# swyoon/Diffusion-by-MaxEntIRL

Measured on AMD Instinct MI355X. Metric: images/sec (CIFAR-10 DDPM T=10 generation), higher is better.
Workload: dtype bf16; 1 GPU; CIFAR-10 DDPM U-Net (35.7M params) VARSampler T=10 generation, 256 images/GPU/step, 3x32x32 (BASELINE configs[1]); noise drawn inside the step; global_batch=256, T=10, parallelism=dp1 (independent trajectories, no collective)

## Files before the change

diffusion-by-maxentirl_amd/csrc/conv_ws.hip:

```cpp
#include "conv_common.h"
#include <stdlib.h>
#include <type_traits>


#ifdef DXMI_CONV_STAMPS
__device__ unsigned g_ws_wait[256][176];
extern "C" int dxmi_debug_read_ws_stamps(void* dst, int bytes) {
    return (int)hipMemcpyFromSymbol(dst, HIP_SYMBOL(g_ws_wait), bytes, 0, hipMemcpyDeviceToHost);
}
#define WS_STAMPED_BARRIER(idx)                                                                     \
    do {                                                                                            \
        const unsigned long long t0_ = __builtin_amdgcn_s_memtime();                                \
        ws_barrier();                                                                               \
        const unsigned long long t1_ = __builtin_amdgcn_s_memtime();                                \
        if (wave == 0 && lane == 0 && (idx) < 160 && blockIdx.x < 256) g_ws_wait[blockIdx.x][(idx)] = (unsigned)(t1_ - t0_); \
    } while (0)
#define WS_CLOCKSTAMP(slot, cond)                                                                    \
    do {                                                                                            \
        if ((cond) && lane == 0 && blockIdx.x < 256) {                                              \
            g_ws_wait[blockIdx.x][(slot)] = (unsigned)__builtin_amdgcn_s_memtime();                 \
            g_ws_wait[blockIdx.x][(slot) + 1] = (unsigned)__builtin_amdgcn_s_memrealtime();         \
        }                                                                                           \
    } while (0)
#define WS_TSTAMP(slot, cond)                                                                        \
    do {                                                                                            \
        if ((cond) && lane == 0 && blockIdx.x < 256) g_ws_wait[blockIdx.x][(slot)] = (unsigned)__builtin_amdgcn_s_memtime(); \
    } while (0)
#define WS_DBG(bit) (p.stagger & (bit))
#else
#define WS_STAMPED_BARRIER(idx) ws_barrier()
#define WS_TSTAMP(slot, cond) do {} while (0)
#define WS_CLOCKSTAMP(slot, cond) do {} while (0)
#define WS_DBG(bit) 0
#endif

__device__ unsigned long long g_ws_clock[4];
extern "C" int dxmi_conv_ws_last_clock(unsigned long long* host_out4) {
    return hipMemcpyFromSymbol(host_out4, HIP_SYMBOL(g_ws_clock), 4 * sizeof(unsigned long long), 0, hipMemcpyDeviceToHost) == hipSuccess ? DXMI_OK
                                                                                                                                          : DXMI_ELAUNCH;
}

namespace {

constexpr int WS_A_SLOT = 8192;
constexpr int WS_RING = 6;
constexpr int WS_A_RING = WS_RING * WS_A_SLOT;
constexpr int WS_RO = 256 * 256;
constexpr int WS_TB = 1024;
constexpr int WS_HALO_BLOCKS = 22;
constexpr int WS_HALO = WS_HALO_BLOCKS * 1024;

__device__ uint4 ws_zero16 = {0u, 0u, 0u, 0u};

#define WS_GPTR(p) ((const __attribute__((address_space(1))) void*)(p))
#define WS_LPTR(p) ((__attribute__((address_space(3))) void*)(p))

__device__ __forceinline__ void ws_barrier() { asm volatile("s_waitcnt lgkmcnt(0)\n\ts_barrier" ::: "memory"); }

#define WS_INTERLEAVE_4()                                       \
    do {                                                        \
        _Pragma("unroll") for (int i_ = 0; i_ < 4; ++i_) {      \
            __builtin_amdgcn_sched_group_barrier(0x008, 3, 0);  \
            __builtin_amdgcn_sched_group_barrier(0x100, 1, 0);  \
        }                                                       \
        __builtin_amdgcn_sched_group_barrier(0x008, 4, 0);      \
    } while (0)
#define WS_INTERLEAVE_8()                                       \
    do {                                                        \
        _Pragma("unroll") for (int i_ = 0; i_ < 8; ++i_) {      \
            __builtin_amdgcn_sched_group_barrier(0x008, 1, 0);  \
            __builtin_amdgcn_sched_group_barrier(0x100, 1, 0);  \
        }                                                       \
        __builtin_amdgcn_sched_group_barrier(0x008, 8, 0);      \
    } while (0)

__device__ __forceinline__ void ws_wait_vm(int n) {
    switch (n >> 1) {
    case 0: asm volatile("s_waitcnt vmcnt(0)" ::: "memory"); break;
    case 1: asm volatile("s_waitcnt vmcnt(2)" ::: "memory"); break;
    case 2: asm volatile("s_waitcnt vmcnt(4)" ::: "memory"); break;
    case 3: asm volatile("s_waitcnt vmcnt(6)" ::: "memory"); break;
    case 4: asm volatile("s_waitcnt vmcnt(8)" ::: "memory"); break;
    case 5: asm volatile("s_waitcnt vmcnt(10)" ::: "memory"); break;
    case 6: asm volatile("s_waitcnt vmcnt(12)" ::: "memory"); break;
    case 7: asm volatile("s_waitcnt vmcnt(14)" ::: "memory"); break;
    case 8: asm volatile("s_waitcnt vmcnt(16)" ::: "memory"); break;
    case 9: asm volatile("s_waitcnt vmcnt(18)" ::: "memory"); break;
    case 10: asm volatile("s_waitcnt vmcnt(20)" ::: "memory"); break;
    default: asm volatile("s_waitcnt vmcnt(22)" ::: "memory"); break;
    }
}

struct WsTile {
    int cot, n0, oy0, ox0;
};

#ifdef WS_VALU_PIECES
typedef float ws_f32x2 __attribute__((ext_vector_type(2)));
struct WsValuLoad {
    u32x4 r[2];
    ws_f32x2 A[4], B[4];
    unsigned sink;
    __device__ __forceinline__ void init(int lane) {
        for (int k = 0; k < 2; ++k) r[k] = u32x4{0x3f803f00u + lane + k, 0xbf803e80u + k, 0x3e003f80u + lane, 0x40003f00u - k};
        for (int i = 0; i < 4; ++i) {
            A[i] = ws_f32x2{0.9f + 0.01f * lane, 1.1f - 0.01f * i};
            B[i] = ws_f32x2{0.05f * i, -0.03f * lane};
        }
        sink = 0;
    }
    __device__ __forceinline__ void run() {
#pragma unroll
        for (int k = 0; k < WS_VALU_PIECES; ++k) {
            u32x4& raw = r[k & 1];
#pragma unroll
            for (int i = 0; i < 4; ++i) {
                ws_f32x2 x = {__builtin_bit_cast(float, raw[i] << 16), __builtin_bit_cast(float, raw[i] & 0xffff0000u)};
                ws_f32x2 y = x * A[i] + B[i];
                const ws_f32x2 t = y * ws_f32x2{-1.4426950408889634f, -1.4426950408889634f};
                ws_f32x2 e = {__builtin_amdgcn_exp2f(t[0]), __builtin_amdgcn_exp2f(t[1])};
                e = e + ws_f32x2{1.f, 1.f};
                const ws_f32x2 rc = {__builtin_amdgcn_rcpf(e[0]), __builtin_amdgcn_rcpf(e[1])};
                y = y * rc;
                bf16x2 o = {(bf16)y[0], (bf16)y[1]};
                sink ^= __builtin_bit_cast(unsigned, o);
            }
            raw += u32x4{0x10001u, 0x20003u, 0x10002u, 0x30001u};
        }
    }
};
#define WS_VALU_DECL(lane_) WsValuLoad vl_; vl_.init(lane_)
#define WS_VALU_RUN() vl_.run()
#define WS_VALU_DONE() do { if (vl_.sink == 0x12345u) reinterpret_cast<volatile unsigned*>(p.out)[0] = vl_.sink; } while (0)
#else
#define WS_VALU_DECL(lane_) do {} while (0)
#define WS_VALU_RUN() do {} while (0)
#define WS_VALU_DONE() do {} while (0)
#endif

template <int TW>
__device__ __forceinline__ void conv_ws_body(const ConvArgs& p) {
    constexpr int TH = 256 / TW, HP = TW == 32 ? 34 : 18, HH = TH + 2, TWl = TW == 32 ? 5 : 4;
    extern __shared__ __attribute__((aligned(1024))) char smem[];
    char* const halo0 = smem;
    char* const aring = smem + 2 * WS_HALO;
    char* const ro = aring + WS_A_RING;
    float* const tb = reinterpret_cast<float*>(ro + WS_RO);

    const int tid = threadIdx.x, lane = tid & 63;
    const int wave = __builtin_amdgcn_readfirstlane(tid >> 6);
    const int txn = p.OW / TW, tyn = p.OH / TH;
    const int nchunks = (p.C0 + p.C1) / 32;
    const int S = 9 * nchunks;
    const int ntiles = p.PT * p.CT;
    const int ups = p.ups ? 1 : 0;

    auto tile_of = [&](int q, WsTile& t) {
        t.cot = q % p.CT;
        const int pt = q / p.CT;
        const int tx = pt % txn, ty = (pt / txn) % tyn;
        t.n0 = pt / (txn * tyn);
        t.oy0 = ty * TH;
        t.ox0 = tx * TW;
    };

    const int q0 = dxmi_xcd_logical(blockIdx.x, gridDim.x, p.xcd_order);
    int q = q0;
    if (q >= ntiles) return;
    const int qstride = gridDim.x;
    if (blockIdx.x == 0 && tid == 0) {
        g_ws_clock[0] = __builtin_amdgcn_s_memtime();
        g_ws_clock[1] = __builtin_amdgcn_s_memrealtime();
    }
    WS_CLOCKSTAMP(172, wave == 0);

    if (wave < 4) {
        const int ch = wave & 1, ph = wave >> 1;
        const int px = lane & 15, kg = lane >> 4;
        constexpr int BROW = TW == 32 ? 2 : 1;
        int bbase[3];
#pragma unroll
        for (int kx = 0; kx < 3; ++kx)
            bbase[kx] = ((ph * (8 / BROW) * HP + px + kx) * 64) + ((kg ^ (2 * (((px + kx) >> 2) & 1))) << 4);
        const char* const abase = aring + ch * 2048 + ((kg >> 1) * 4096) + ((px + 32 * (kg & 1)) << 4);
        f32x4 acc[4][8];
#pragma unroll
        for (int cb = 0; cb < 4; ++cb)
#pragma unroll
            for (int nb = 0; nb < 8; ++nb)
#pragma unroll
                for (int r = 0; r < 4; ++r) acc[cb][nb][r] = 0.f;
        bf16x8 A0[4], A1[4], Bx[4], By[4];
        auto read_a = [&](int u, bf16x8 (&A)[4]) {
            const char* as = abase + (u % WS_RING) * WS_A_SLOT;
#pragma unroll
            for (int cb = 0; cb < 4; ++cb) A[cb] = *reinterpret_cast<const bf16x8*>(as + (cb >> 1) * 1024 + (cb & 1) * 256);
        };
        auto read_b = [&](int u, int half, bf16x8 (&B)[4]) {
            const int t = u % 9, ky = t / 3, kx = t % 3;
            const char* hb = halo0 + ((u / 9) & 1) * WS_HALO + bbase[kx];
#pragma unroll
            for (int i = 0; i < 4; ++i) {
                const int nb = half * 4 + i;
                B[i] = *reinterpret_cast<const bf16x8*>(hb + ((nb / BROW + ky) * HP + (nb % BROW) * 16) * 64);
            }
        };
        auto mfma16 = [&](const bf16x8 (&A)[4], const bf16x8 (&B)[4], int half) {
#pragma unroll
            for (int i = 0; i < 4; ++i)
#pragma unroll
                for (int cb = 0; cb < 4; ++cb)
                    acc[cb][half * 4 + i] = __builtin_amdgcn_mfma_f32_16x16x32_bf16(A[cb], B[i], acc[cb][half * 4 + i], 0, 0, 0);
        };
        const float slope = dxmi_act_slope(p.act);
        const bool has_res = p.residual != nullptr;

        ws_barrier();
        WS_CLOCKSTAMP(168, wave == 0);
        read_a(0, A0);
        read_b(0, 0, Bx);
        int stamp_i = 0;
        (void)stamp_i;
        for (;;) {
            const bool more = q + qstride < ntiles;
            for (int c = 0; c < nchunks; c += 2) {
#pragma unroll
                for (int u = 0; u < 18; ++u) {
                    read_b(u, 1, By);
                    if (u & 1) mfma16(A1, Bx, 0); else mfma16(A0, Bx, 0);
                    WS_INTERLEAVE_4();
                    if (u % 3 == 2) { if (!(WS_DBG(16))) WS_STAMPED_BARRIER(stamp_i + c * 9 + u); }
                    if (u & 1) read_a(u + 1, A0); else read_a(u + 1, A1);
                    read_b(u + 1, 0, Bx);
                    if (u & 1) mfma16(A1, By, 1); else mfma16(A0, By, 1);
                    WS_INTERLEAVE_8();
                    __builtin_amdgcn_sched_barrier(0);
                }
            }
            WS_TSTAMP(158, wave == 0 && q == q0);
            ws_barrier();
            WS_TSTAMP(159, wave == 0 && q == q0);
            {
                const bool plain = p.act == DXMI_ACT_NONE;
                char* const rowb = ro + ((ph * 128 + px) << 8) + 8 * (kg & 1);
                const bool want_stats = p.gn_stats != nullptr;
                const int cot_ = q % p.CT;
                float* const stp = want_stats ? p.gn_stats + ((size_t)((q / p.CT) * 2 + ph) * (p.Cout >> 1) + cot_ * 64 + ch * 32 + kg * 2) * 2 : nullptr;
                auto epi = [&](auto RES, auto MASK, auto ACT, auto STATS) {
                    constexpr bool kRes = decltype(RES)::value, kMask = decltype(MASK)::value, kAct = decltype(ACT)::value, kStats = decltype(STATS)::value;
#pragma unroll
                    for (int cb = 0; cb < 4; ++cb) {
                        float st[4] = {0.f, 0.f, 0.f, 0.f};
                        const int co = ch * 64 + cb * 16 + 4 * kg;
                        const f32x4 b0 = *reinterpret_cast<const f32x4*>(tb + co), t0 = *reinterpret_cast<const f32x4*>(tb + 128 + co);
                        f32x4 bv;
#pragma unroll
                        for (int e = 0; e < 4; ++e) bv[e] = b0[e] + t0[e];
                        char* const a0 = rowb + (((ch * 8 + cb * 2 + (kg >> 1)) ^ px) << 4);
                        bf16x4 r[8];
                        if constexpr (kRes) {
#pragma unroll
                            for (int nb = 0; nb < 8; ++nb) r[nb] = *reinterpret_cast<const bf16x4*>(a0 + nb * 4096);
                        }
#pragma unroll
                        for (int nb = 0; nb < 8; ++nb) {
                            f32x4 v;
#pragma unroll
                            for (int e = 0; e < 4; ++e) v[e] = acc[cb][nb][e] + bv[e];
                            if constexpr (kRes) {
                                if constexpr (kMask) {
#pragma unroll
                                    for (int e = 0; e < 4; ++e) v[e] *= ((float)r[nb][e] > 0.f ? 1.f : p.mask_slope);
                                } else {
#pragma unroll
                                    for (int e = 0; e < 4; ++e) v[e] += (float)r[nb][e];
                                }
                            }
                            if constexpr (kAct) {
#pragma unroll
                                for (int e = 0; e < 4; ++e) v[e] = dxmi_act_lin(v[e], slope);
                            }
                            bf16x4 o;
#pragma unroll
                            for (int e = 0; e < 4; ++e) o[e] = (bf16)v[e];
                            *reinterpret_cast<bf16x4*>(a0 + nb * 4096) = o;
                            if constexpr (kStats) dxmi_stats4(o, st);
#pragma unroll
                            for (int e = 0; e < 4; ++e) acc[cb][nb][e] = 0.f;
                        }
                        if constexpr (kStats) {
#pragma unroll
                            for (int e = 0; e < 4; ++e) st[e] = dxmi_row16_sum(st[e]);
                            if (px == 0 && cot_ * 128 + co < p.Cout) {
                                f32x4 sv;
#pragma unroll
                                for (int e = 0; e < 4; ++e) sv[e] = st[e];
                                *reinterpret_cast<f32x4*>(stp + cb * 16) = sv;
                            }
                        }
                    }
                };
                using T_ = std::true_type;
                using F_ = std::false_type;
                const bool is_mask = has_res && p.res_is_mask;
                if (plain && !is_mask) {
                    if (has_res) { if (want_stats) epi(T_{}, F_{}, F_{}, T_{}); else epi(T_{}, F_{}, F_{}, F_{}); }
                    else { if (want_stats) epi(F_{}, F_{}, F_{}, T_{}); else epi(F_{}, F_{}, F_{}, F_{}); }
                } else if (!want_stats) {
                    if (is_mask) { if (plain) epi(T_{}, T_{}, F_{}, F_{}); else epi(T_{}, T_{}, T_{}, F_{}); }
                    else if (has_res) epi(T_{}, F_{}, T_{}, F_{});
                    else epi(F_{}, F_{}, T_{}, F_{});
                } else {
                    if (is_mask) epi(T_{}, T_{}, T_{}, T_{});
                    else if (has_res) epi(T_{}, F_{}, T_{}, T_{});
                    else epi(F_{}, F_{}, T_{}, T_{});
                }
            }
            WS_TSTAMP(166, wave == 0 && q == q0);
            ws_barrier();
            WS_TSTAMP(157, wave == 0 && q == q0);
// ... 50 lines not shown
        if (WS_DBG(1)) {}
        const int t2l = lw * 64 + lane, prl = t2l >> 4;
        const int lpar_l0 = prl * p.Cout + (((t2l & 15) ^ prl) * 8), lpar_l1 = prl * p.Cout + (((t2l & 15) ^ (prl | 8)) * 8);
        const int c8e_l = (t2l & 15) ^ prl, c8o_l = (t2l & 15) ^ (prl | 8);
        const int kpc_l = (32 + nchunks - 2) / (nchunks - 1);
        const char* const zero_page_l = reinterpret_cast<const char*>(p.mask_src);
        bool first_tile_l = true, first_group0 = true;
        load_group(0, cur.cot, cur.cot, fq[0]);
        load_group(1, cur.cot, cur.cot, fq[1]);
        asm volatile("s_waitcnt vmcnt(12)" ::: "memory");
        store_group(0, fq[0]);
        asm volatile("s_waitcnt lgkmcnt(0)" ::: "memory");
        load_group(2, cur.cot, cur.cot, fq[0]);
        ws_barrier();
        bool first_tile = true;
        for (;;) {
            const bool more = q + qstride < ntiles;
            WsTile nxt = cur;
            if (more) tile_of(q + qstride, nxt);
            if (!first_tile && lw == 0 && !(WS_DBG(8))) {
                const int co_a = cur.cot * 128 + lane, co_b = co_a + 64 < p.Cout ? co_a + 64 : p.Cout - 1;
                if (p.bias) {
                    __builtin_amdgcn_global_load_lds(WS_GPTR(p.bias + co_a), WS_LPTR(tb), 4, 0, 0);
                    __builtin_amdgcn_global_load_lds(WS_GPTR(p.bias + co_b), WS_LPTR(tb + 64), 4, 0, 0);
                }
                if (p.addvec) {
                    const float* av = p.addvec + (size_t)cur.n0 * p.addvec_ld;
                    __builtin_amdgcn_global_load_lds(WS_GPTR(av + co_a), WS_LPTR(tb + 128), 4, 0, 0);
                    __builtin_amdgcn_global_load_lds(WS_GPTR(av + co_b), WS_LPTR(tb + 192), 4, 0, 0);
                }
            }
            const bf16* const res_t = p.residual + ((((size_t)cur.n0 * p.OH + cur.oy0) * p.OW + cur.ox0) * p.Cout + cur.cot * 128);
            const bool res_here = !first_tile_l && p.residual != nullptr && !(WS_DBG(8));
            first_tile_l = false;
            first_tile = false;
            for (int G0 = 0; G0 < NG; G0 += 2) {
#pragma unroll
                for (int j = 0; j < 2; ++j) {
                    const int G = G0 + j;
                    if (G > 0 || first_group0) {
                        asm volatile("s_waitcnt vmcnt(12)" ::: "memory");
                        store_group(G + 1, fq[(j + 1) & 1]);
                        asm volatile("s_waitcnt lgkmcnt(0)" ::: "memory");
                    }
                    if (res_here && G > 0) {
                        const int cg = (G - 1) / 3, g3 = (G - 1) - cg * 3;
                        if (cg + 1 < nchunks) {
                            const int k0 = cg * kpc_l < 32 ? cg * kpc_l : 32, k1 = k0 + kpc_l < 32 ? k0 + kpc_l : 32;
                            const int i0 = g3 < 2 ? 3 * g3 : 6, i1 = g3 < 2 ? 3 * g3 + 3 : 12;
                            const int ka = k0 + i0 < k1 ? k0 + i0 : k1, kb = k0 + i1 < k1 ? k0 + i1 : k1;
#pragma unroll 1
                            for (int k = ka; k < kb; ++k) {
                                const int rel = ((k >> (TWl - 3)) * p.OW + (k & (TW / 8 - 1)) * 8) * p.Cout + ((k & 1) ? lpar_l1 : lpar_l0);
                                const bool ok = cur.cot * 128 + ((k & 1) ? c8o_l : c8e_l) * 8 < p.Cout;
                                const void* g = ok ? (const void*)(res_t + rel) : (const void*)zero_page_l;
                                __builtin_amdgcn_global_load_lds(WS_GPTR(g), WS_LPTR(ro + (k * 128 + lw * 64) * 16), 16, 0, 0);
                            }
                        }
                    }
                    if (G > 0 || first_group0) load_group(G + 3, cur.cot, more ? nxt.cot : cur.cot, fq[(j + 1) & 1]);
                    WS_TSTAMP(151, wave == 4 && G == 0 && q == q0 + qstride);
                    WS_VALU_RUN();
                    if (!(WS_DBG(16))) ws_barrier();
                }
            }
            first_group0 = false;
            if (more) {
                asm volatile("s_waitcnt vmcnt(12)" ::: "memory");
                store_group(1, fq[1]);
                asm volatile("s_waitcnt lgkmcnt(0)" ::: "memory");
                load_group(3, nxt.cot, nxt.cot, fq[1]);
            }
            ws_barrier();
            ws_barrier();
            WS_TSTAMP(150, wave == 4 && q == q0);
            if (!more) break;
            q += qstride;
            cur = nxt;
        }
        asm volatile("s_waitcnt vmcnt(0)" ::: "memory");
        WS_VALU_DONE();
    } else if (wave == 6) {
        WS_VALU_DECL(lane);
        constexpr int HBA = WS_HALO_BLOCKS;
        const char* const zero_page = reinterpret_cast<const char*>(p.mask_src);
        int hrel0[HBA], hrel1[HBA];
        unsigned m_in = 0, m_top = 0, m_bot = 0, m_left = 0, m_right = 0;
#pragma unroll
        for (int k = 0; k < HBA; ++k) {
            const int hp = k * 16 + (lane >> 2);
            const int hy = hp / HP, hx = hp - hy * HP;
            const int rel = ((hy - 1) >> ups) * p.IW + ((hx - 1) >> ups);
            const int j8 = ((lane & 3) ^ (2 * ((hx >> 2) & 1))) * 8;
            hrel0[k] = (rel * p.C0 + j8) * 2;
            hrel1[k] = (rel * p.C1 + j8) * 2;
            m_in |= (unsigned)(hy < HH && hx < TW + 2) << k;
            m_top |= (unsigned)(hy == 0) << k;
            m_bot |= (unsigned)(hy == HH - 1) << k;
            m_left |= (unsigned)(hx == 0) << k;
            m_right |= (unsigned)(hx == TW + 1) << k;
        }
        unsigned hmask = 0;
        int hbase0 = 0, hbase1 = 0;
        auto halo_plan = [&](const WsTile& t) {
            hmask = m_in;
            if (t.oy0 == 0) hmask &= ~m_top;
            if (t.oy0 + TH == p.OH) hmask &= ~m_bot;
            if (t.ox0 == 0) hmask &= ~m_left;
            if (t.ox0 + TW == p.OW) hmask &= ~m_right;
            const int pix = (t.n0 * p.IH + (t.oy0 >> ups)) * p.IW + (t.ox0 >> ups);
            hbase0 = pix * p.C0 * 2;
            hbase1 = pix * p.C1 * 2;
        };
        auto halo_issue = [&](int c, char* buf, int ka, int kb) {
            if (WS_DBG(2)) return;
            const int cbase = c * 32;
            const bool first = cbase < p.C0;
            const char* base = reinterpret_cast<const char*>(first ? p.in0 : p.in1) + (first ? cbase : cbase - p.C0) * 2 + (first ? hbase0 : hbase1);
#pragma unroll
            for (int k = 0; k < HBA; ++k) {
                if (k < ka || k >= kb) continue;
                const char* g = (hmask >> k) & 1 ? base + (first ? hrel0[k] : hrel1[k]) : zero_page;
                __builtin_amdgcn_global_load_lds(WS_GPTR(g), WS_LPTR(buf + k * 1024), 16, 0, 0);
            }
        };
        WsTile cur;
        tile_of(q, cur);
        if (!p.bias) { tb[lane] = 0.f; tb[64 + lane] = 0.f; }
        if (!p.addvec) { tb[128 + lane] = 0.f; tb[192 + lane] = 0.f; }
        halo_plan(cur);
        halo_issue(0, halo0, 0, HBA);
        if (!(WS_DBG(8))) {
            const int co_a = cur.cot * 128 + lane, co_b = co_a + 64 < p.Cout ? co_a + 64 : p.Cout - 1;
            if (p.bias) {
                __builtin_amdgcn_global_load_lds(WS_GPTR(p.bias + co_a), WS_LPTR(tb), 4, 0, 0);
                __builtin_amdgcn_global_load_lds(WS_GPTR(p.bias + co_b), WS_LPTR(tb + 64), 4, 0, 0);
            }
            if (p.addvec) {
                const float* av = p.addvec + (size_t)cur.n0 * p.addvec_ld;
                __builtin_amdgcn_global_load_lds(WS_GPTR(av + co_a), WS_LPTR(tb + 128), 4, 0, 0);
                __builtin_amdgcn_global_load_lds(WS_GPTR(av + co_b), WS_LPTR(tb + 192), 4, 0, 0);
            }
        }
        asm volatile("s_waitcnt vmcnt(0)" ::: "memory");
        ws_barrier();
        WsTile nxt = cur;
        for (;;) {
            const bool more = q + qstride < ntiles;
            for (int c = 0; c < nchunks; ++c) {
                const bool wrap = c + 1 == nchunks;
                if (wrap && more) {
                    tile_of(q + qstride, nxt);
                    halo_plan(nxt);
                }
                const bool do_halo = !wrap || more;
                char* const hbuf = halo0 + ((c + 1) & 1) * WS_HALO;
                const int hc = wrap ? 0 : c + 1;
#pragma unroll
                for (int t = 0; t < 9; ++t) {
                    if (t < 8 && do_halo) halo_issue(hc, hbuf, 3 * t, 3 * t + 3 < HBA ? 3 * t + 3 : HBA);
                    if (t == 8) asm volatile("s_waitcnt vmcnt(0)" ::: "memory");
                    if (t % 3 == 2) { WS_VALU_RUN(); if (!(WS_DBG(16))) ws_barrier(); }
                }
            }
            ws_barrier();
            ws_barrier();
            if (!more) break;
            q += qstride;
            cur = nxt;
        }
        WS_VALU_DONE();
    } else if (wave == 7) {
        WS_VALU_DECL(lane);
        const char* const zero_page = reinterpret_cast<const char*>(p.mask_src);
        const int prA = lane >> 4, prB = 4 + (lane >> 4), lc = lane & 15;
        const int lparA[2] = {prA * p.Cout + ((lc ^ prA) * 8), prA * p.Cout + ((lc ^ (prA | 8)) * 8)};
        const int lparB[2] = {prB * p.Cout + ((lc ^ prB) * 8), prB * p.Cout + ((lc ^ (prB | 8)) * 8)};
        const int c8A[2] = {lc ^ prA, lc ^ (prA | 8)}, c8B[2] = {lc ^ prB, lc ^ (prB | 8)};
        auto tile_base = [&](const WsTile& t) -> size_t {
            return (((size_t)t.n0 * p.OH + t.oy0) * p.OW + t.ox0) * p.Cout + t.cot * 128;
        };
        auto piece_u = [&](int k) -> int { return ((k >> (TWl - 3)) * p.OW + (k & (TW / 8 - 1)) * 8) * p.Cout; };
        WsTile cur;
        tile_of(q, cur);
        if (p.residual != nullptr && !(WS_DBG(8))) {
            const bf16* rb = p.residual + tile_base(cur);
#pragma unroll 1
            for (int k = 0; k < 32; ++k) {
                const int u = piece_u(k);
                const void* ga = cur.cot * 128 + c8A[k & 1] * 8 < p.Cout ? (const void*)(rb + u + lparA[k & 1]) : (const void*)zero_page;
                const void* gb = cur.cot * 128 + c8B[k & 1] * 8 < p.Cout ? (const void*)(rb + u + lparB[k & 1]) : (const void*)zero_page;
                __builtin_amdgcn_global_load_lds(WS_GPTR(ga), WS_LPTR(ro + (k * 128) * 16), 16, 0, 0);
                __builtin_amdgcn_global_load_lds(WS_GPTR(gb), WS_LPTR(ro + (k * 128 + 64) * 16), 16, 0, 0);
            }
        }
        ws_barrier();
        bool have_prev = false;
        WsTile prev = cur;
        const int kpc = (32 + nchunks - 2) / (nchunks - 1);
        auto piece_range = [&](int c, int t, int& ka, int& kb) {
            ka = kb = 32;
            if (!have_prev || c + 1 >= nchunks) return;
            const int k0 = c * kpc < 32 ? c * kpc : 32, k1 = k0 + kpc < 32 ? k0 + kpc : 32;
            const int i0 = t < 6 ? t : 6 + 2 * (t - 6), i1 = t < 6 ? t + 1 : i0 + 2;
            ka = k0 + i0 < k1 ? k0 + i0 : k1;
            kb = k0 + i1 < k1 ? k0 + i1 : k1;
        };
        const bool do_drain = !(WS_DBG(4));
        bf16* out_prev = reinterpret_cast<bf16*>(p.out);
        for (;;) {
            const bool more = q + qstride < ntiles;
            WsTile nxt = cur;
            if (more) tile_of(q + qstride, nxt);
            for (int c = 0; c < nchunks; ++c) {
#pragma unroll
                for (int t = 0; t < 9; ++t) {
                    int ka, kb;
                    piece_range(c, t, ka, kb);
                    if (ka < kb && do_drain) {
                        bf16x8 va[2], vb[2];
#pragma unroll
                        for (int u = 0; u < 2; ++u)
                            if (ka + u < kb) {
                                va[u] = *reinterpret_cast<const bf16x8*>(ro + ((ka + u) * 128 + lane) * 16);
                                vb[u] = *reinterpret_cast<const bf16x8*>(ro + ((ka + u) * 128 + 64 + lane) * 16);
                            }
#pragma unroll
                        for (int u = 0; u < 2; ++u)
                            if (ka + u < kb) {
                                const int k = ka + u, pu = piece_u(k);
                                if (prev.cot * 128 + c8A[k & 1] * 8 < p.Cout) *reinterpret_cast<bf16x8*>(out_prev + pu + lparA[k & 1]) = va[u];
                                if (prev.cot * 128 + c8B[k & 1] * 8 < p.Cout) *reinterpret_cast<bf16x8*>(out_prev + pu + lparB[k & 1]) = vb[u];
                            }
                    }
                    asm volatile("s_waitcnt lgkmcnt(0)" ::: "memory");
                    if (t % 3 == 2) { WS_VALU_RUN(); if (!(WS_DBG(16))) ws_barrier(); }
                }
            }
            if (!have_prev) asm volatile("s_waitcnt vmcnt(0)" ::: "memory");
            ws_barrier();
            ws_barrier();
            out_prev = reinterpret_cast<bf16*>(p.out) + tile_base(cur);
            prev = cur;
// ... 95 lines not shown
```

diffusion-by-maxentirl_amd/csrc/conv_ws8.hip:

```cpp
#include "conv_common.h"
#include <stdlib.h>
#include <type_traits>


namespace {

constexpr int W8_ROW = 8 * 64;
constexpr int W8_IMG = 10 * W8_ROW;
constexpr int W8_HALO_BLOCKS = 16;
constexpr int W8_HALO = 4 * W8_IMG;
constexpr int W8_STRIP = W8_IMG;
constexpr int W8_A_SLOT = 4096;
#ifndef W8_RING_SLOTS
#define W8_RING_SLOTS 6
#endif
constexpr int W8_RING = W8_RING_SLOTS;
constexpr int W8_A_RING = W8_RING * W8_A_SLOT;
constexpr int W8_RO = 256 * 128;
constexpr int W8_TB = 2048;

__device__ uint4 w8_zero16 = {0u, 0u, 0u, 0u};

#ifdef DXMI_CONV_STAMPS
#define W8_DBG(bit) (p.stagger & (bit))
#else
#define W8_DBG(bit) 0
#endif

#define W8_GPTR(p) ((const __attribute__((address_space(1))) void*)(p))
#define W8_LPTR(p) ((__attribute__((address_space(3))) void*)(p))

__device__ __forceinline__ void w8_barrier() { asm volatile("s_waitcnt lgkmcnt(0)\n\ts_barrier" ::: "memory"); }

#define W8_INTERLEAVE_2()                                       \
    do {                                                        \
        _Pragma("unroll") for (int i_ = 0; i_ < 2; ++i_) {      \
            __builtin_amdgcn_sched_group_barrier(0x008, 3, 0);  \
            __builtin_amdgcn_sched_group_barrier(0x100, 1, 0);  \
        }                                                       \
        __builtin_amdgcn_sched_group_barrier(0x008, 2, 0);      \
    } while (0)
#define W8_INTERLEAVE_6()                                       \
    do {                                                        \
        _Pragma("unroll") for (int i_ = 0; i_ < 6; ++i_) {      \
            __builtin_amdgcn_sched_group_barrier(0x008, 1, 0);  \
            __builtin_amdgcn_sched_group_barrier(0x100, 1, 0);  \
        }                                                       \
        __builtin_amdgcn_sched_group_barrier(0x008, 2, 0);      \
    } while (0)

__device__ __forceinline__ void w8_wait_vm(int n) {
    switch (n >> 1) {
    case 0: asm volatile("s_waitcnt vmcnt(0)" ::: "memory"); break;
    case 1: asm volatile("s_waitcnt vmcnt(2)" ::: "memory"); break;
    case 2: asm volatile("s_waitcnt vmcnt(4)" ::: "memory"); break;
    case 3: asm volatile("s_waitcnt vmcnt(6)" ::: "memory"); break;
    case 4: asm volatile("s_waitcnt vmcnt(8)" ::: "memory"); break;
    case 5: asm volatile("s_waitcnt vmcnt(10)" ::: "memory"); break;
    default: asm volatile("s_waitcnt vmcnt(12)" ::: "memory"); break;
    }
}

struct W8Tile {
    int cot, n0;
};

template <bool GN>
__global__ __launch_bounds__(512, 1) void conv_ws8_kernel(ConvArgs p) {
    extern __shared__ __attribute__((aligned(1024))) char smem[];
    char* const halo0 = smem;
    char* const aring = smem + 2 * W8_HALO + W8_STRIP;
    char* const ro = aring + W8_A_RING;
    float* const tb = reinterpret_cast<float*>(ro + W8_RO);

    const int tid = threadIdx.x, lane = tid & 63;
    const int wave = __builtin_amdgcn_readfirstlane(tid >> 6);
    const int nchunks = (p.C0 + p.C1) / 32;
    const int S = 9 * nchunks;
    const int ntiles = p.PT * p.CT;

    auto tile_of = [&](int q, W8Tile& t) {
        t.cot = q % p.CT;
        t.n0 = (q / p.CT) * 4;
    };

    int q = dxmi_xcd_logical(blockIdx.x, gridDim.x, p.xcd_order);
    if (q >= ntiles) return;
    const int qstride = gridDim.x;

    if (wave < 4) {
        const int px = lane & 15, kg = lane >> 4;
        int bbase[2][3];
#pragma unroll
        for (int kx = 0; kx < 3; ++kx) {
            const int col = (px & 7) + kx - 1;
            const int low = (px >> 3) * W8_ROW + ((kg ^ ((col & 4) >> 1)) << 4);
            const bool inside = col >= 0 && col < 8;
#pragma unroll
            for (int b = 0; b < 2; ++b)
                bbase[b][kx] = inside ? b * W8_HALO + wave * W8_IMG + col * 64 + low : 2 * W8_HALO + (col & 3) * 64 + low;
        }
        const char* const abase = aring + ((kg >> 1) * 2048) + ((px + 32 * (kg & 1)) << 4);
        f32x4 acc[4][4];
#pragma unroll
        for (int cb = 0; cb < 4; ++cb)
#pragma unroll
            for (int nb = 0; nb < 4; ++nb)
#pragma unroll
                for (int r = 0; r < 4; ++r) acc[cb][nb][r] = 0.f;
        bf16x8 A0[4], A1[4], Bx[2], By[2];
        auto read_a = [&](int u, bf16x8 (&A)[4]) {
            const char* as = abase + (u % W8_RING) * W8_A_SLOT;
#pragma unroll
            for (int cb = 0; cb < 4; ++cb) A[cb] = *reinterpret_cast<const bf16x8*>(as + (cb >> 1) * 1024 + (cb & 1) * 256);
        };
        auto read_b = [&](int u, int half, bf16x8 (&B)[2]) {
            const int t = u % 9, ky = t / 3, kx = t % 3;
            const char* hb = halo0 + bbase[(u / 9) & 1][kx];
#pragma unroll
            for (int i = 0; i < 2; ++i) B[i] = *reinterpret_cast<const bf16x8*>(hb + (2 * (half * 2 + i) + ky) * W8_ROW);
        };
        auto mfma8 = [&](const bf16x8 (&A)[4], const bf16x8 (&B)[2], int half) {
#pragma unroll
            for (int i = 0; i < 2; ++i)
#pragma unroll
                for (int cb = 0; cb < 4; ++cb)
                    acc[cb][half * 2 + i] = __builtin_amdgcn_mfma_f32_16x16x32_bf16(A[cb], B[i], acc[cb][half * 2 + i], 0, 0, 0);
        };
        const float slope = dxmi_act_slope(p.act);
        const bool has_res = p.residual != nullptr;

        {
            const uint4 z = {0u, 0u, 0u, 0u};
#pragma unroll
            for (int b = 0; b < 2; ++b)
                *reinterpret_cast<uint4*>(halo0 + b * W8_HALO + wave * W8_IMG + (lane >> 5) * 9 * W8_ROW + (lane & 31) * 16) = z;
            for (int i = wave; i < W8_STRIP / 1024; i += 4) *reinterpret_cast<uint4*>(halo0 + 2 * W8_HALO + i * 1024 + lane * 16) = z;
        }
        w8_barrier();
        read_a(0, A0);
        read_b(0, 0, Bx);
        for (;;) {
            const bool more = q + qstride < ntiles;
            f32x4 gam[4], bet[4];
            if constexpr (GN) {
                const int co0 = (q % p.CT) * 64 + 4 * kg;
#pragma unroll
                for (int cb = 0; cb < 4; ++cb) {
                    gam[cb] = *reinterpret_cast<const f32x4*>(p.gn_gamma + co0 + cb * 16);
                    bet[cb] = *reinterpret_cast<const f32x4*>(p.gn_beta + co0 + cb * 16);
                }
            }
            for (int c = 0; c < nchunks; c += 2) {
#pragma unroll
                for (int u = 0; u < 18; ++u) {
                    read_b(u, 1, By);
                    if (u & 1) mfma8(A1, Bx, 0); else mfma8(A0, Bx, 0);
                    W8_INTERLEAVE_2();
                    if (u % 3 == 2 && !(W8_DBG(4))) w8_barrier();
                    if (u & 1) read_a(u + 1, A0); else read_a(u + 1, A1);
                    read_b(u + 1, 0, Bx);
                    if (u & 1) mfma8(A1, By, 1); else mfma8(A0, By, 1);
                    W8_INTERLEAVE_6();
                    __builtin_amdgcn_sched_barrier(0);
                }
            }
            w8_barrier();
            {
                const bool plain = p.act == DXMI_ACT_NONE;
                char* const rowb = ro + ((wave * 64 + px) << 7) + 8 * (kg & 1);
                auto epi = [&](auto RES, auto MASK, auto ACT) {
                    constexpr bool kRes = decltype(RES)::value, kMask = decltype(MASK)::value, kAct = decltype(ACT)::value;
#pragma unroll
                    for (int cb = 0; cb < 4; ++cb) {
                        const int co = cb * 16 + 4 * kg;
                        const f32x4 b0 = *reinterpret_cast<const f32x4*>(tb + co), t0 = *reinterpret_cast<const f32x4*>(tb + 64 + wave * 64 + co);
                        f32x4 bv;
#pragma unroll
                        for (int e = 0; e < 4; ++e) bv[e] = b0[e] + t0[e];
                        char* const a0 = rowb + (((cb * 2 + (kg >> 1)) ^ (px & 7)) << 4);
                        bf16x4 r[4];
                        if constexpr (kRes) {
#pragma unroll
                            for (int nb = 0; nb < 4; ++nb) r[nb] = *reinterpret_cast<const bf16x4*>(a0 + nb * 2048);
                        }
#pragma unroll
                        for (int nb = 0; nb < 4; ++nb) {
                            f32x4 v;
#pragma unroll
                            for (int e = 0; e < 4; ++e) v[e] = acc[cb][nb][e] + bv[e];
                            if constexpr (kRes) {
                                if constexpr (kMask) {
#pragma unroll
                                    for (int e = 0; e < 4; ++e) v[e] *= ((float)r[nb][e] > 0.f ? 1.f : p.mask_slope);
                                } else {
#pragma unroll
                                    for (int e = 0; e < 4; ++e) v[e] += (float)r[nb][e];
                                }
                            }
                            if constexpr (kAct) {
#pragma unroll
                                for (int e = 0; e < 4; ++e) v[e] = dxmi_act_lin(v[e], slope);
                            }
                            bf16x4 o;
#pragma unroll
                            for (int e = 0; e < 4; ++e) o[e] = (bf16)v[e];
                            if constexpr (GN) {
#pragma unroll
                                for (int e = 0; e < 4; ++e) acc[cb][nb][e] = (float)o[e];
                            } else {
                                *reinterpret_cast<bf16x4*>(a0 + nb * 2048) = o;
#pragma unroll
                                for (int e = 0; e < 4; ++e) acc[cb][nb][e] = 0.f;
                            }
                        }
                        if constexpr (GN) {
                            float s = 0.f;
#pragma unroll
                            for (int nb = 0; nb < 4; ++nb) s += (acc[cb][nb][0] + acc[cb][nb][1]) + (acc[cb][nb][2] + acc[cb][nb][3]);
                            s = dxmi_row16_sum(s);
                            s += __shfl_xor(s, 16, 64);
                            const float mean = s * (1.f / 512.f);
                            float qv = 0.f;
#pragma unroll
                            for (int nb = 0; nb < 4; ++nb) {
                                float d[4];
#pragma unroll
                                for (int e = 0; e < 4; ++e) d[e] = acc[cb][nb][e] - mean;
                                qv += (d[0] * d[0] + d[1] * d[1]) + (d[2] * d[2] + d[3] * d[3]);
                            }
                            qv = dxmi_row16_sum(qv);
                            qv += __shfl_xor(qv, 16, 64);
                            const float rstd = rsqrtf(qv * (1.f / 512.f) + p.gn_eps);
                            float ga[4], be[4];
#pragma unroll
                            for (int e = 0; e < 4; ++e) {
                                ga[e] = gam[cb][e] * rstd;
                                be[e] = bet[cb][e] - mean * ga[e];
                            }
#pragma unroll
                            for (int nb = 0; nb < 4; ++nb) {
                                bf16x4 y;
#pragma unroll
                                for (int e = 0; e < 4; ++e) {
                                    float t = acc[cb][nb][e] * ga[e] + be[e];
                                    if (p.gn_flags & 1) t = dxmi_silu_fast(t);
                                    y[e] = (bf16)t;
                                    acc[cb][nb][e] = 0.f;
// ... 322 lines not shown
```

Baseline: 6870 images/s.

## Compact TW=16 halo layout, pre-zero padding once, batch halo loads

```diff
diff --git a/diffusion-by-maxentirl_amd/csrc/conv_ws.hip b/diffusion-by-maxentirl_amd/csrc/conv_ws.hip
--- a/diffusion-by-maxentirl_amd/csrc/conv_ws.hip
+++ b/diffusion-by-maxentirl_amd/csrc/conv_ws.hip
@@ -49,6 +49,14 @@
 constexpr int WS_TB = 1024;
 constexpr int WS_HALO_BLOCKS = 22;
 constexpr int WS_HALO = WS_HALO_BLOCKS * 1024;
+#ifndef WS_H32_A
+#define WS_H32_A 11
+#define WS_H32_B 22
+#endif
+#ifndef WS_H16_A
+#define WS_H16_A 9
+#define WS_H16_B 18
+#endif
 
 __device__ uint4 ws_zero16 = {0u, 0u, 0u, 0u};
 
@@ -140,7 +148,7 @@
 
 template <int TW>
 __device__ __forceinline__ void conv_ws_body(const ConvArgs& p) {
-    constexpr int TH = 256 / TW, HP = TW == 32 ? 34 : 18, HH = TH + 2, TWl = TW == 32 ? 5 : 4;
+    constexpr int TH = 256 / TW, HP = TW == 32 ? 34 : 17, HH = TH + 2, TWl = TW == 32 ? 5 : 4;
     extern __shared__ __attribute__((aligned(1024))) char smem[];
     char* const halo0 = smem;
     char* const aring = smem + 2 * WS_HALO;
@@ -452,14 +460,17 @@
         WS_VALU_DONE();
     } else if (wave == 6) {
         WS_VALU_DECL(lane);
-        constexpr int HBA = WS_HALO_BLOCKS;
+        constexpr bool T16 = TW == 16;
+        constexpr int HBA = T16 ? HH : WS_HALO_BLOCKS;
+        constexpr int HSA = T16 ? WS_H16_A : WS_H32_A, HSB = T16 ? WS_H16_B : WS_H32_B;
+        const bool pad_rows_stay = T16 && p.OH == TH;
         const char* const zero_page = reinterpret_cast<const char*>(p.mask_src);
         int hrel0[HBA], hrel1[HBA];
         unsigned m_in = 0, m_top = 0, m_bot = 0, m_left = 0, m_right = 0;
 #pragma unroll
         for (int k = 0; k < HBA; ++k) {
             const int hp = k * 16 + (lane >> 2);
-            const int hy = hp / HP, hx = hp - hy * HP;
+            const int hy = T16 ? k : hp / HP, hx = T16 ? 1 + (lane >> 2) : hp - hy * HP;
             const int rel = ((hy - 1) >> ups) * p.IW + ((hx - 1) >> ups);
             const int j8 = ((lane & 3) ^ (2 * ((hx >> 2) & 1))) * 8;
             hrel0[k] = (rel * p.C0 + j8) * 2;
@@ -490,14 +501,27 @@
 #pragma unroll
             for (int k = 0; k < HBA; ++k) {
                 if (k < ka || k >= kb) continue;
+                if (T16 && (k == 0 || k == HBA - 1) && pad_rows_stay) continue;
                 const char* g = (hmask >> k) & 1 ? base + (first ? hrel0[k] : hrel1[k]) : zero_page;
-                __builtin_amdgcn_global_load_lds(WS_GPTR(g), WS_LPTR(buf + k * 1024), 16, 0, 0);
+                __builtin_amdgcn_global_load_lds(WS_GPTR(g), WS_LPTR(buf + (T16 ? (k * HP + 1) * 64 : k * 1024)), 16, 0, 0);
             }
         };
         WsTile cur;
         tile_of(q, cur);
         if (!p.bias) { tb[lane] = 0.f; tb[64 + lane] = 0.f; }
         if (!p.addvec) { tb[128 + lane] = 0.f; tb[192 + lane] = 0.f; }
+        if constexpr (T16) {
+#pragma unroll
+            for (int i = 0; i < 7; ++i) {
+                const int s = i * 64 + lane;
+                if (s < 416) {
+                    const int b = s >= 208 ? 1 : 0, r = s - b * 208, pz = r >> 2;
+                    const int pix = pz < 18 ? pz : pz < 36 ? (HH - 1) * HP - 18 + pz : (pz - 35) * HP;
+                    *reinterpret_cast<u32x4*>(halo0 + b * WS_HALO + pix * 64 + (r & 3) * 16) = u32x4{0u, 0u, 0u, 0u};
+                }
+            }
+            asm volatile("s_waitcnt lgkmcnt(0)" ::: "memory");
+        }
         halo_plan(cur);
         halo_issue(0, halo0, 0, HBA);
         if (!(WS_DBG(8))) {
@@ -528,7 +552,11 @@
                 const int hc = wrap ? 0 : c + 1;
 #pragma unroll
                 for (int t = 0; t < 9; ++t) {
-                    if (t < 8 && do_halo) halo_issue(hc, hbuf, 3 * t, 3 * t + 3 < HBA ? 3 * t + 3 : HBA);
+                    if (do_halo) {
+                        if (t == 0) halo_issue(hc, hbuf, 0, HSA);
+                        if (t == 3) halo_issue(hc, hbuf, HSA, HSB);
+                        if (t == 6) halo_issue(hc, hbuf, HSB, HBA);
+                    }
                     if (t == 8) asm volatile("s_waitcnt vmcnt(0)" ::: "memory");
                     if (t % 3 == 2) { WS_VALU_RUN(); if (!(WS_DBG(16))) ws_barrier(); }
                 }
```

Result: no change. 6888 images/s, median of 6 (+0.3%).

## Hand-schedule LDS reads and MFMAs with explicit lgkmcnt waits in conv mainloops

Applied to the files above, without the earlier changes.

```diff
diff --git a/diffusion-by-maxentirl_amd/csrc/conv_ws.hip b/diffusion-by-maxentirl_amd/csrc/conv_ws.hip
--- a/diffusion-by-maxentirl_amd/csrc/conv_ws.hip
+++ b/diffusion-by-maxentirl_amd/csrc/conv_ws.hip
@@ -1,6 +1,7 @@
 #include "conv_common.h"
 #include <stdlib.h>
 #include <type_traits>
+#include <utility>
 
 
 #ifdef DXMI_CONV_STAMPS
@@ -8,10 +9,10 @@
 extern "C" int dxmi_debug_read_ws_stamps(void* dst, int bytes) {
     return (int)hipMemcpyFromSymbol(dst, HIP_SYMBOL(g_ws_wait), bytes, 0, hipMemcpyDeviceToHost);
 }
-#define WS_STAMPED_BARRIER(idx)                                                                     \
+#define WS_STAMPED_BARRIER(idx, barrier_fn)                                                         \
     do {                                                                                            \
         const unsigned long long t0_ = __builtin_amdgcn_s_memtime();                                \
-        ws_barrier();                                                                               \
+        barrier_fn();                                                                               \
         const unsigned long long t1_ = __builtin_amdgcn_s_memtime();                                \
         if (wave == 0 && lane == 0 && (idx) < 160 && blockIdx.x < 256) g_ws_wait[blockIdx.x][(idx)] = (unsigned)(t1_ - t0_); \
     } while (0)
@@ -28,7 +29,7 @@
     } while (0)
 #define WS_DBG(bit) (p.stagger & (bit))
 #else
-#define WS_STAMPED_BARRIER(idx) ws_barrier()
+#define WS_STAMPED_BARRIER(idx, barrier_fn) barrier_fn()
 #define WS_TSTAMP(slot, cond) do {} while (0)
 #define WS_CLOCKSTAMP(slot, cond) do {} while (0)
 #define WS_DBG(bit) 0
@@ -57,22 +58,37 @@
 
 __device__ __forceinline__ void ws_barrier() { asm volatile("s_waitcnt lgkmcnt(0)\n\ts_barrier" ::: "memory"); }
 
-#define WS_INTERLEAVE_4()                                       \
-    do {                                                        \
-        _Pragma("unroll") for (int i_ = 0; i_ < 4; ++i_) {      \
-            __builtin_amdgcn_sched_group_barrier(0x008, 3, 0);  \
-            __builtin_amdgcn_sched_group_barrier(0x100, 1, 0);  \
-        }                                                       \
-        __builtin_amdgcn_sched_group_barrier(0x008, 4, 0);      \
+#if defined(DXMI_WS_GROUP_DRAIN) || defined(DXMI_CONV_STAMPS)
+__device__ __forceinline__ void ws_barrier_inflight() { ws_barrier(); }
+#else
+__device__ __forceinline__ void ws_barrier_inflight() { asm volatile("s_barrier" ::: "memory"); }
+#endif
+
+#define WS_PIN() __builtin_amdgcn_sched_barrier(0)
+#define WS_LDS_ADDR(p) ((unsigned)(size_t)WS_LPTR(p))
+#define WS_RD(dst, addr, off)                                                                             \
+    do {                                                                                                  \
+        WS_PIN();                                                                                         \
+        asm volatile("ds_read_b128 %0, %1 offset:%2" : "=v"(dst) : "v"(addr), "i"(off));                  \
+        WS_PIN();                                                                                         \
     } while (0)
-#define WS_INTERLEAVE_8()                                       \
-    do {                                                        \
-        _Pragma("unroll") for (int i_ = 0; i_ < 8; ++i_) {      \
-            __builtin_amdgcn_sched_group_barrier(0x008, 1, 0);  \
-            __builtin_amdgcn_sched_group_barrier(0x100, 1, 0);  \
-        }                                                       \
-        __builtin_amdgcn_sched_group_barrier(0x008, 8, 0);      \
+#define WS_WAIT1(n, b)                                                                                    \
+    do {                                                                                                  \
+        WS_PIN();                                                                                         \
+        asm volatile("s_waitcnt lgkmcnt(" #n ")" : "+v"(b));                                              \
+        WS_PIN();                                                                                         \
     } while (0)
+#define WS_WAIT5(n, A, b)                                                                                 \
+    do {                                                                                                  \
+        WS_PIN();                                                                                         \
+        asm volatile("s_waitcnt lgkmcnt(" #n ")" : "+v"(A[0]), "+v"(A[1]), "+v"(A[2]), "+v"(A[3]), "+v"(b)); \
+        WS_PIN();                                                                                         \
+    } while (0)
+
+template <int... I, class F>
+__device__ __forceinline__ void ws_static_for(std::integer_sequence<int, I...>, F&& f) {
+    (f(std::integral_constant<int, I>{}), ...);
+}
 
 __device__ __forceinline__ void ws_wait_vm(int n) {
     switch (n >> 1) {
@@ -191,51 +207,75 @@
 #pragma unroll
                 for (int r = 0; r < 4; ++r) acc[cb][nb][r] = 0.f;
         bf16x8 A0[4], A1[4], Bx[4], By[4];
-        auto read_a = [&](int u, bf16x8 (&A)[4]) {
-            const char* as = abase + (u % WS_RING) * WS_A_SLOT;
-#pragma unroll
-            for (int cb = 0; cb < 4; ++cb) A[cb] = *reinterpret_cast<const bf16x8*>(as + (cb >> 1) * 1024 + (cb & 1) * 256);
-        };
-        auto read_b = [&](int u, int half, bf16x8 (&B)[4]) {
-            const int t = u % 9, ky = t / 3, kx = t % 3;
-            const char* hb = halo0 + ((u / 9) & 1) * WS_HALO + bbase[kx];
-#pragma unroll
-            for (int i = 0; i < 4; ++i) {
-                const int nb = half * 4 + i;
-                B[i] = *reinterpret_cast<const bf16x8*>(hb + ((nb / BROW + ky) * HP + (nb % BROW) * 16) * 64);
-            }
-        };
-        auto mfma16 = [&](const bf16x8 (&A)[4], const bf16x8 (&B)[4], int half) {
-#pragma unroll
-            for (int i = 0; i < 4; ++i)
-#pragma unroll
-                for (int cb = 0; cb < 4; ++cb)
-                    acc[cb][half * 4 + i] = __builtin_amdgcn_mfma_f32_16x16x32_bf16(A[cb], B[i], acc[cb][half * 4 + i], 0, 0, 0);
-        };
+        const unsigned a_lds = WS_LDS_ADDR(abase);
+        unsigned b_lds[3];
+#pragma unroll
+        for (int kx = 0; kx < 3; ++kx) b_lds[kx] = WS_LDS_ADDR(halo0) + bbase[kx];
+#define WS_RD_A(A, u_, cb_) WS_RD(A[cb_], a_lds, ((u_) % WS_RING) * WS_A_SLOT + ((cb_) >> 1) * 1024 + ((cb_) & 1) * 256)
+#define WS_RD_B(B, u_, half_, i_)                                                                        \
+    WS_RD(B[i_], b_lds[((u_) % 9) % 3],                                                                  \
+          (((u_) / 9) & 1) * WS_HALO + ((((half_) * 4 + (i_)) / BROW + ((u_) % 9) / 3) * HP + (((half_) * 4 + (i_)) % BROW) * 16) * 64)
+#define WS_MFMA(A, B, half_, i_, cb_) \
+    acc[cb_][(half_) * 4 + (i_)] = __builtin_amdgcn_mfma_f32_16x16x32_bf16(A[cb_], B[i_], acc[cb_][(half_) * 4 + (i_)], 0, 0, 0)
+#define WS_MFMA4(A, B, half_, i_)                                                                        \
+    do {                                                                                                 \
+        WS_MFMA(A, B, half_, i_, 0); WS_MFMA(A, B, half_, i_, 1); WS_MFMA(A, B, half_, i_, 2); WS_MFMA(A, B, half_, i_, 3); \
+    } while (0)
         const float slope = dxmi_act_slope(p.act);
         const bool has_res = p.residual != nullptr;
 
         ws_barrier();
         WS_CLOCKSTAMP(168, wave == 0);
-        read_a(0, A0);
-        read_b(0, 0, Bx);
+        WS_RD_A(A0, 0, 0); WS_RD_A(A0, 0, 1); WS_RD_A(A0, 0, 2); WS_RD_A(A0, 0, 3);
+        WS_RD_B(Bx, 0, 0, 0); WS_RD_B(Bx, 0, 0, 1); WS_RD_B(Bx, 0, 0, 2); WS_RD_B(Bx, 0, 0, 3);
         int stamp_i = 0;
         (void)stamp_i;
         for (;;) {
             const bool more = q + qstride < ntiles;
             for (int c = 0; c < nchunks; c += 2) {
-#pragma unroll
-                for (int u = 0; u < 18; ++u) {
-                    read_b(u, 1, By);
-                    if (u & 1) mfma16(A1, Bx, 0); else mfma16(A0, Bx, 0);
-                    WS_INTERLEAVE_4();
-                    if (u % 3 == 2) { if (!(WS_DBG(16))) WS_STAMPED_BARRIER(stamp_i + c * 9 + u); }
-                    if (u & 1) read_a(u + 1, A0); else read_a(u + 1, A1);
-                    read_b(u + 1, 0, Bx);
-                    if (u & 1) mfma16(A1, By, 1); else mfma16(A0, By, 1);
-                    WS_INTERLEAVE_8();
-                    __builtin_amdgcn_sched_barrier(0);
-                }
+                auto step = [&](auto U) {
+                    constexpr int u = decltype(U)::value;
+                    bf16x8 (&A)[4] = (u & 1) ? A1 : A0;
+                    bf16x8 (&An)[4] = (u & 1) ? A0 : A1;
+                    WS_WAIT5(3, A, Bx[0]);
+                    WS_MFMA(A, Bx, 0, 0, 0); WS_MFMA(A, Bx, 0, 0, 1); WS_MFMA(A, Bx, 0, 0, 2);
+                    WS_RD_B(By, u, 1, 0);
+                    WS_MFMA(A, Bx, 0, 0, 3);
+                    WS_WAIT1(3, Bx[1]);
+                    WS_MFMA(A, Bx, 0, 1, 0); WS_MFMA(A, Bx, 0, 1, 1);
+                    WS_RD_B(By, u, 1, 1);
+                    WS_MFMA(A, Bx, 0, 1, 2); WS_MFMA(A, Bx, 0, 1, 3);
+                    WS_WAIT1(3, Bx[2]);
+                    WS_MFMA(A, Bx, 0, 2, 0);
+                    WS_RD_B(By, u, 1, 2);
+                    WS_MFMA(A, Bx, 0, 2, 1); WS_MFMA(A, Bx, 0, 2, 2); WS_MFMA(A, Bx, 0, 2, 3);
+                    WS_RD_B(By, u, 1, 3);
+                    WS_WAIT1(4, Bx[3]);
+                    WS_MFMA4(A, Bx, 0, 3);
+                    WS_PIN();
+                    if constexpr (u % 3 == 2) {
+                        if (!(WS_DBG(16))) {
+                            if constexpr (u % 9 == 8) WS_STAMPED_BARRIER(stamp_i + c * 9 + u, ws_barrier);
+                            else WS_STAMPED_BARRIER(stamp_i + c * 9 + u, ws_barrier_inflight);
+                        }
+                    }
+                    WS_WAIT1(3, By[0]);
+                    WS_MFMA(A, By, 1, 0, 0); WS_RD_A(An, u + 1, 0);
+                    WS_MFMA(A, By, 1, 0, 1); WS_RD_A(An, u + 1, 1);
+                    WS_MFMA(A, By, 1, 0, 2); WS_RD_A(An, u + 1, 2);
+                    WS_MFMA(A, By, 1, 0, 3); WS_RD_A(An, u + 1, 3);
+                    WS_WAIT1(6, By[1]);
+                    WS_MFMA(A, By, 1, 1, 0); WS_RD_B(Bx, u + 1, 0, 0);
+                    WS_MFMA(A, By, 1, 1, 1); WS_RD_B(Bx, u + 1, 0, 1);
+                    WS_MFMA(A, By, 1, 1, 2); WS_RD_B(Bx, u + 1, 0, 2);
+                    WS_MFMA(A, By, 1, 1, 3); WS_RD_B(Bx, u + 1, 0, 3);
+                    WS_WAIT1(9, By[2]);
+                    WS_MFMA4(A, By, 1, 2);
+                    WS_WAIT1(8, By[3]);
+                    WS_MFMA4(A, By, 1, 3);
+                    WS_PIN();
+                };
+                ws_static_for(std::make_integer_sequence<int, 18>{}, step);
             }
             WS_TSTAMP(158, wave == 0 && q == q0);
             ws_barrier();
diff --git a/diffusion-by-maxentirl_amd/csrc/conv_ws8.hip b/diffusion-by-maxentirl_amd/csrc/conv_ws8.hip
--- a/diffusion-by-maxentirl_amd/csrc/conv_ws8.hip
+++ b/diffusion-by-maxentirl_amd/csrc/conv_ws8.hip
@@ -1,6 +1,7 @@
 #include "conv_common.h"
 #include <stdlib.h>
 #include <type_traits>
+#include <utility>
 
 
 namespace {
@@ -32,22 +33,37 @@
 
 __device__ __forceinline__ void w8_barrier() { asm volatile("s_waitcnt lgkmcnt(0)\n\ts_barrier" ::: "memory"); }
 
-#define W8_INTERLEAVE_2()                                       \
-    do {                                                        \
-        _Pragma("unroll") for (int i_ = 0; i_ < 2; ++i_) {      \
-            __builtin_amdgcn_sched_group_barrier(0x008, 3, 0);  \
-            __builtin_amdgcn_sched_group_barrier(0x100, 1, 0);  \
-        }                                                       \
-        __builtin_amdgcn_sched_group_barrier(0x008, 2, 0);      \
+#ifdef DXMI_WS_GROUP_DRAIN
+__device__ __forceinline__ void w8_barrier_inflight() { w8_barrier(); }
+#else
+__device__ __forceinline__ void w8_barrier_inflight() { asm volatile("s_barrier" ::: "memory"); }
+#endif
+
+#define W8_PIN() __builtin_amdgcn_sched_barrier(0)
+#define W8_LDS_ADDR(p) ((unsigned)(size_t)W8_LPTR(p))
+#define W8_RD(dst, addr, off)                                                                             \
+    do {                                                                                                  \
+        W8_PIN();                                                                                         \
+        asm volatile("ds_read_b128 %0, %1 offset:%2" : "=v"(dst) : "v"(addr), "i"(off));                  \
+        W8_PIN();                                                                                         \
     } while (0)
-#define W8_INTERLEAVE_6()                                       \
-    do {                                                        \
-        _Pragma("unroll") for (int i_ = 0; i_ < 6; ++i_) {      \
-            __builtin_amdgcn_sched_group_barrier(0x008, 1, 0);  \
-            __builtin_amdgcn_sched_group_barrier(0x100, 1, 0);  \
-        }                                                       \
-        __builtin_amdgcn_sched_group_barrier(0x008, 2, 0);      \
+#define W8_WAIT1(n, b)                                                                                    \
+    do {                                                                                                  \
+        W8_PIN();                                                                                         \
+        asm volatile("s_waitcnt lgkmcnt(" #n ")" : "+v"(b));                                              \
+        W8_PIN();                                                                                         \
     } while (0)
+#define W8_WAIT5(n, A, b)                                                                                 \
+    do {                                                                                                  \
+        W8_PIN();                                                                                         \
+        asm volatile("s_waitcnt lgkmcnt(" #n ")" : "+v"(A[0]), "+v"(A[1]), "+v"(A[2]), "+v"(A[3]), "+v"(b)); \
+        W8_PIN();                                                                                         \
+    } while (0)
+
+template <int... I, class F>
+__device__ __forceinline__ void w8_static_for(std::integer_sequence<int, I...>, F&& f) {
+    (f(std::integral_constant<int, I>{}), ...);
+}
 
 __device__ __forceinline__ void w8_wait_vm(int n) {
     switch (n >> 1) {
@@ -109,24 +125,16 @@
 #pragma unroll
                 for (int r = 0; r < 4; ++r) acc[cb][nb][r] = 0.f;
         bf16x8 A0[4], A1[4], Bx[2], By[2];
-        auto read_a = [&](int u, bf16x8 (&A)[4]) {
-            const char* as = abase + (u % W8_RING) * W8_A_SLOT;
-#pragma unroll
-            for (int cb = 0; cb < 4; ++cb) A[cb] = *reinterpret_cast<const bf16x8*>(as + (cb >> 1) * 1024 + (cb & 1) * 256);
-        };
-        auto read_b = [&](int u, int half, bf16x8 (&B)[2]) {
-            const int t = u % 9, ky = t / 3, kx = t % 3;
-            const char* hb = halo0 + bbase[(u / 9) & 1][kx];
-#pragma unroll
-            for (int i = 0; i < 2; ++i) B[i] = *reinterpret_cast<const bf16x8*>(hb + (2 * (half * 2 + i) + ky) * W8_ROW);
-        };
-        auto mfma8 = [&](const bf16x8 (&A)[4], const bf16x8 (&B)[2], int half) {
-#pragma unroll
-            for (int i = 0; i < 2; ++i)
-#pragma unroll
-                for (int cb = 0; cb < 4; ++cb)
-                    acc[cb][half * 2 + i] = __builtin_amdgcn_mfma_f32_16x16x32_bf16(A[cb], B[i], acc[cb][half * 2 + i], 0, 0, 0);
-        };
+        const unsigned a_lds = W8_LDS_ADDR(abase);
+        unsigned b_lds[2][3];
+#pragma unroll
+        for (int b = 0; b < 2; ++b)
+#pragma unroll
+            for (int kx = 0; kx < 3; ++kx) b_lds[b][kx] = W8_LDS_ADDR(halo0) + bbase[b][kx];
+#define W8_RD_A(A, u_, cb_) W8_RD(A[cb_], a_lds, ((u_) % W8_RING) * W8_A_SLOT + ((cb_) >> 1) * 1024 + ((cb_) & 1) * 256)
+#define W8_RD_B(B, u_, half_, i_) W8_RD(B[i_], b_lds[((u_) / 9) & 1][((u_) % 9) % 3], (2 * ((half_) * 2 + (i_)) + ((u_) % 9) / 3) * W8_ROW)
+#define W8_MFMA(A, B, half_, i_, cb_) \
+    acc[cb_][(half_) * 2 + (i_)] = __builtin_amdgcn_mfma_f32_16x16x32_bf16(A[cb_], B[i_], acc[cb_][(half_) * 2 + (i_)], 0, 0, 0)
         const float slope = dxmi_act_slope(p.act);
         const bool has_res = p.residual != nullptr;
 
@@ -138,8 +146,8 @@
             for (int i = wave; i < W8_STRIP / 1024; i += 4) *reinterpret_cast<uint4*>(halo0 + 2 * W8_HALO + i * 1024 + lane * 16) = z;
         }
         w8_barrier();
-        read_a(0, A0);
-        read_b(0, 0, Bx);
+        W8_RD_A(A0, 0, 0); W8_RD_A(A0, 0, 1); W8_RD_A(A0, 0, 2); W8_RD_A(A0, 0, 3);
+        W8_RD_B(Bx, 0, 0, 0); W8_RD_B(Bx, 0, 0, 1);
         for (;;) {
             const bool more = q + qstride < ntiles;
             f32x4 gam[4], bet[4];
@@ -152,18 +160,37 @@
                 }
             }
             for (int c = 0; c < nchunks; c += 2) {
-#pragma unroll
-                for (int u = 0; u < 18; ++u) {
-                    read_b(u, 1, By);
-                    if (u & 1) mfma8(A1, Bx, 0); else mfma8(A0, Bx, 0);
-                    W8_INTERLEAVE_2();
-                    if (u % 3 == 2 && !(W8_DBG(4))) w8_barrier();
-                    if (u & 1) read_a(u + 1, A0); else read_a(u + 1, A1);
-                    read_b(u + 1, 0, Bx);
-                    if (u & 1) mfma8(A1, By, 1); else mfma8(A0, By, 1);
-                    W8_INTERLEAVE_6();
-                    __builtin_amdgcn_sched_barrier(0);
-                }
+                auto step = [&](auto U) {
+                    constexpr int u = decltype(U)::value;
+                    bf16x8 (&A)[4] = (u & 1) ? A1 : A0;
+                    bf16x8 (&An)[4] = (u & 1) ? A0 : A1;
+                    W8_WAIT5(1, A, Bx[0]);
+                    W8_MFMA(A, Bx, 0, 0, 0); W8_MFMA(A, Bx, 0, 0, 1); W8_MFMA(A, Bx, 0, 0, 2);
+                    W8_RD_B(By, u, 1, 0);
+                    W8_MFMA(A, Bx, 0, 0, 3);
+                    W8_WAIT1(1, Bx[1]);
+                    W8_MFMA(A, Bx, 0, 1, 0); W8_MFMA(A, Bx, 0, 1, 1);
+                    W8_RD_B(By, u, 1, 1);
+                    W8_MFMA(A, Bx, 0, 1, 2); W8_MFMA(A, Bx, 0, 1, 3);
+                    W8_PIN();
+                    if constexpr (u % 3 == 2) {
+                        if (!(W8_DBG(4))) {
+                            if constexpr (u % 9 == 8) w8_barrier();
+                            else w8_barrier_inflight();
+                        }
+                    }
+                    W8_WAIT1(1, By[0]);
+                    W8_MFMA(A, By, 1, 0, 0); W8_RD_A(An, u + 1, 0);
+                    W8_MFMA(A, By, 1, 0, 1); W8_RD_A(An, u + 1, 1);
+                    W8_MFMA(A, By, 1, 0, 2); W8_RD_A(An, u + 1, 2);
+                    W8_MFMA(A, By, 1, 0, 3); W8_RD_A(An, u + 1, 3);
+                    W8_WAIT1(4, By[1]);
+                    W8_MFMA(A, By, 1, 1, 0); W8_RD_B(Bx, u + 1, 0, 0);
+                    W8_MFMA(A, By, 1, 1, 1); W8_RD_B(Bx, u + 1, 0, 1);
+                    W8_MFMA(A, By, 1, 1, 2); W8_MFMA(A, By, 1, 1, 3);
+                    W8_PIN();
+                };
+                w8_static_for(std::make_integer_sequence<int, 18>{}, step);
             }
             w8_barrier();
             {
```

After: 6948 images/s before, 6996 images/s after, median of 6. About the same (+0.7%).
